# QuanjianSong/UniVST

Hardware: AMD Instinct MI355X
Metric: stylized frames/sec, SD-v1.5 16x512x512 @50 DDIM steps (higher is better)
Workload: dtype f16; 1 GPU; sd15_unet_three_branch_pnp_transfer_16x512x512_50ddim; frames=16, branches=3, schedule_steps=54 (wrapping modulo 50), masks=moving disc, blended on steps 0..45, parallelism=single, weights=random-init SD-v1.5 architecture (859M + 201M temporal params), fp16

## Files before the change

### univst_amd/csrc/attention.hip

```cpp
#include "common.h"

#include "kernels.h"

namespace {

constexpr int KT = 64;
constexpr float DEFER = 8.f;

typedef __fp16 fh2 __attribute__((ext_vector_type(2)));

__device__ __forceinline__ float max3f(float a, float b, float c) {
    float r;
    asm("v_max3_f32 %0, %1, %2, %3" : "=v"(r) : "v"(a), "v"(b), "v"(c));
    return r;
}

__device__ __forceinline__ void attn_merge_coef(float m1, float l1, float m2, float l2, float& w1, float& w2) {
    const bool has1 = l1 > 0.f, has2 = l2 > 0.f;
    const float m = has1 ? (has2 ? fmaxf(m1, m2) : m1) : m2;
    const float a1 = has1 ? l1 * __builtin_amdgcn_exp2f(m1 - m) : 0.f;
    const float a2 = has2 ? __builtin_amdgcn_exp2f(m2 - m) : 0.f;
    const float den = a1 + l2 * a2;
    const float inv = den > 0.f ? 1.f / den : 0.f;
    w1 = a1 * inv;
// ... 721 lines not shown
#define UV_PP_PHASE2()                                                            \
    _Pragma("unroll") for (int i_ = 0; i_ < 12; ++i_) {                           \
        __builtin_amdgcn_sched_group_barrier(0x008, 1, 0);                        \
        if (i_ < 4) __builtin_amdgcn_sched_group_barrier(0x100, 1, 0);            \
        __builtin_amdgcn_sched_group_barrier(0x002, 2, 0);                        \
    }

#define UV_PP_PIN4(a) asm volatile("" : "+v"(a[0]), "+v"(a[1]), "+v"(a[2]), "+v"(a[3]))
#define UV_PP_PIN2(a, i) asm volatile("" : "+v"(a[i]), "+v"(a[(i) + 1]))

    if (STG) {
        dma_tile(0);
        if (T > 1) dma_tile(TILE);
        asm volatile("s_waitcnt vmcnt(0)" ::: "memory");
    } else {
        load_tile();
        store_tile(smem);
        if (T > 1) {
            load_tile();
            store_tile(smem + TILE);
        }
    }
    __syncthreads();

    f4 scA[2][QB], scB[2][QB];
    h8 kf[2][2], vf[DV16], pb[QB];
    float mx[QB];
    int nx_s = 0, nx_t = (ntile > 1) ? 1 : 0;
    if (ntile == 1) nx_s = 1;
    float lw_nxt = (nx_s != 0 && nx_s < nsrc_eff && p.src_logw) ? p.src_logw[bf * p.nsrc + nx_s] : lw_cur;
    int t0_cur = 0, t0_nxt = nx_t * KT;
    half_t* b_cur = smem;
    half_t* b_nxt = smem + TILE;
    half_t* b_ld = smem + 2 * TILE;

    kfrag_read(b_cur, 0, kf);
    qk(kf, scA);
    if (t0_cur + KT > p.Nkv) mask_tail(scA, t0_cur);
    local_max(scA, mx);
    decide(scA, mx, true);
    kfrag_read(b_cur, 1, kf);

    for (int tt = 0; tt < T; ++tt) {
        const bool has_next = tt + 1 < T;
        if (tt + 2 < T) {
            if (STG) dma_tile((int)(b_ld - smem));
            else load_tile();
        }
        vfrag_read(b_cur, 0, vf);
        if (K16) {
            qk_a(kf, scB);
            exp_half(scA, pb, 0);
            UV_PP_PIN2(pb, 0);
            UV_PP_PHASE1H(1);
            qk_fence(scB);
            __builtin_amdgcn_sched_barrier(0);
            qk_b(kf, scB);
            exp_half(scA, pb, 1);
            UV_PP_PIN2(pb, 2);
            UV_PP_PHASE1H(0);
        } else {
            qk(kf, scB);
            exp_part(scA, pb);
            UV_PP_PIN4(pb);
            UV_PP_PHASE1();
        }
        __builtin_amdgcn_sched_barrier(0);
        if (t0_cur + KT > p.Nkv) mask_tail(scB, t0_cur + 32);
        kfrag_read(b_nxt, 0, kf);
        pv(vf, pb);
        local_max(scB, mx);
        UV_PP_PIN4(mx);
        UV_PP_PHASE2();
        __builtin_amdgcn_sched_barrier(0);
        decide(scB, mx, false);
        if (lw_nxt != lw_cur) set_lw(lw_nxt);
        vfrag_read(b_cur, 1, vf);
        if (K16) {
            qk_a(kf, scA);
            exp_half(scB, pb, 0);
            UV_PP_PIN2(pb, 0);
            UV_PP_PHASE1H(1);
            qk_fence(scA);
            __builtin_amdgcn_sched_barrier(0);
            qk_b(kf, scA);
            exp_half(scB, pb, 1);
            UV_PP_PIN2(pb, 2);
            UV_PP_PHASE1H(0);
        } else {
            qk(kf, scA);
            exp_part(scB, pb);
            UV_PP_PIN4(pb);
            UV_PP_PHASE1();
        }
        __builtin_amdgcn_sched_barrier(0);
        if (has_next && t0_nxt + KT > p.Nkv) mask_tail(scA, t0_nxt);
        kfrag_read(b_nxt, 1, kf);
        pv(vf, pb);
        local_max(scA, mx);
        UV_PP_PIN4(mx);
        UV_PP_PHASE2();
        __builtin_amdgcn_sched_barrier(0);
        if (has_next) decide(scA, mx, false);
        if (!STG && tt + 2 < T) store_tile(b_ld);
        if (STG) asm volatile("s_waitcnt vmcnt(0)" ::: "memory");
        __syncthreads();
        half_t* tb = b_cur; b_cur = b_nxt; b_nxt = b_ld; b_ld = tb;
        t0_cur = t0_nxt;
        lw_cur = lw_nxt;
        if (++nx_t == ntile) {
            nx_t = 0;
            if (++nx_s < nsrc_eff && p.src_logw) lw_nxt = p.src_logw[bf * p.nsrc + nx_s];
        }
        t0_nxt = nx_t * KT;
    }
#undef UV_PP_PHASE1
#undef UV_PP_PHASE1H
#undef UV_PP_PIN2
#undef UV_PP_PIN4
#undef UV_PP_PHASE2

#pragma unroll
    for (int qb = 0; qb < QB; ++qb) {
        const float l = __shfl(o[DV16 - 1][qb][0], 32 + l15, 64);
        float inv = 1.f / l, w1 = 0.f;
        const int qrow = qblk * 64 * NW + wave * 16 * QB + qb * 16 + l15;
        if (qrow >= p.Nq) continue;
        half_t* op = p.o + ((long)bf * p.Nq + qrow) * p.ldo + h * D;
        if constexpr (TP != 0) {
            const float m2 = mrun[qb];
            const long srow = (((long)bf * p.heads + h) * p.Nq + qrow) * 2;
            if constexpr (TP == 1) {
                if (g == 0) *reinterpret_cast<float2*>(p.state_out + srow) = make_float2(m2, l);
            } else {
                const float2 st = *reinterpret_cast<const float2*>(p.state_in + srow);
                attn_merge_coef(st.x, st.y, m2, l, w1, inv);
            }
        }
#pragma unroll
        for (int dv = 0; dv < DV16; ++dv) {
            const int dc = dv * 16 + g * 4;
            if (dc < D) {
                h4 ov;
                if constexpr (TP == 2) {
                    const h4 o1 = *reinterpret_cast<const h4*>(op + dc);
#pragma unroll
                    for (int r = 0; r < 4; ++r) ov[r] = (half_t)fmaf((float)o1[r], w1, o[dv][qb][r] * inv);
                } else {
#pragma unroll
                    for (int r = 0; r < 4; ++r) ov[r] = (half_t)(o[dv][qb][r] * inv);
                }
                *reinterpret_cast<h4*>(op + dc) = ov;
            }
        }
    }
}

template <int TAG = 0, int TP = 0>
__global__ __launch_bounds__(256, 2) void attn_pp64_kernel(AttnParams p) {
    constexpr int D = 64, QB = 4;
    constexpr int NW = 4, DV16 = D / 16, NST = 3;
    constexpr int KS = D / 32;
    constexpr int NDK = D / 8, NPV = D / 8;
    constexpr int RB = NW * 16 * QB;
    constexpr int KPL = 512, VPL = 576;
    constexpr int KAREA = NDK * KPL;
    constexpr int TILE = NDK * KPL + NPV * VPL;
    __shared__ __attribute__((aligned(16))) half_t smem[NST * TILE];

    const int tid = threadIdx.x, lane = tid & 63, wave = tid >> 6;
    const int l15 = lane & 15, g = lane >> 4;
    const int nqb = (p.Nq + RB - 1) / RB;
    const int lid = xcd_remap(blockIdx.x, gridDim.x);
    const int qblk = lid % nqb;
    const int h = p.order ? lid / (nqb * p.BF) : (lid / nqb) % p.heads;
    const int bf = p.order ? (lid / nqb) % p.BF : lid / (nqb * p.heads);
    const h8 zero8 = {0, 0, 0, 0, 0, 0, 0, 0};

    const int ntile = (p.Nkv + KT - 1) / KT;
    const int ntile_x = p.kx ? (p.Nkv_x + KT - 1) / KT : 0;
    const int nsrc_eff = p.src_cnt ? p.src_cnt[bf] : p.nsrc;
    const int nseg = nsrc_eff + (p.kx ? 1 : 0);
    const int T = nsrc_eff * ntile + ntile_x;
    if (TP && T == 0) {
        attn_empty_phase<NW * 16 * QB>(p, bf, h, qblk, D);
        return;
    }
    auto seg_lw = [&](int sidx) { return (sidx < nsrc_eff && p.src_logw) ? p.src_logw[bf * p.nsrc + sidx] : 0.f; };
    auto seg_nkv = [&](int sidx) { return sidx < nsrc_eff ? p.Nkv : p.Nkv_x; };
    auto seg_ntile = [&](int sidx) { return sidx < nsrc_eff ? ntile : ntile_x; };

    h8 qf[QB][KS];
#pragma unroll
    for (int qb = 0; qb < QB; ++qb) {
        const int qrow = qblk * RB + wave * 16 * QB + qb * 16 + l15;
#pragma unroll
        for (int ks = 0; ks < KS; ++ks)
            qf[qb][ks] = (qrow < p.Nq && ks * 32 + g * 8 < D) ? *reinterpret_cast<const h8*>(p.q + ((long)bf * p.Nq + qrow) * p.ldq + h * D + ks * 32 + g * 8) : zero8;
    }

    f4 o[DV16][QB], cfold[QB];
    float mrun[QB], lsum[QB];
    float lw_cur = seg_lw(0);
#pragma unroll
    for (int qb = 0; qb < QB; ++qb) {
        mrun[qb] = 0.f;
        lsum[qb] = 0.f;
        cfold[qb] = f4{lw_cur, lw_cur, lw_cur, lw_cur};
#pragma unroll
        for (int dv = 0; dv < DV16; ++dv) o[dv][qb] = f4{0.f, 0.f, 0.f, 0.f};
    }

    const int wave_u = __builtin_amdgcn_readfirstlane(wave);
    const half_t* const zpage = uv_attn_zero_page;
    const unsigned smem_lds = (unsigned)(size_t)((__attribute__((address_space(3))) half_t*)smem);
    auto glds16 = [](const half_t* src, unsigned lds_byte) {
        unsigned keep;
        asm volatile("s_mov_b32 %0, m0\n\ts_mov_b32 m0, %2\n\ts_nop 0\n\tglobal_load_lds_dwordx4 %1, off\n\ts_mov_b32 m0, %0"
                     : "=&s"(keep) : "v"(src), "s"(lds_byte) : "memory");
    };
    const long xk_delta = p.kx ? (long)(p.kx - p.k) : 0, xv_delta = p.kx ? (long)(p.vx - p.v) : 0;
    int ld_s = 0, ld_t = 0;
    long ld_koff, ld_voff, ld_ld;
    int ld_nkv, ld_ntile;
    {
        const long off = (long)__builtin_amdgcn_readfirstlane(p.src_idx[bf * p.nsrc]) * p.Nkv * p.ldkv + h * D;
        ld_koff = off; ld_voff = off; ld_ld = p.ldkv; ld_nkv = p.Nkv; ld_ntile = ntile;
    }
    auto dma_tile = [&](int stage_half) {
        const int t0 = ld_t * KT;
        const bool rok = t0 + lane < ld_nkv;
        const long roff = (long)(t0 + lane) * ld_ld;
        const half_t* const ksrc = p.k + ld_koff + roff;
        const half_t* const vsrc = p.v + ld_voff + roff;
#pragma unroll
        for (int j = 0; j < (NDK + NPV + NW - 1) / NW; ++j) {
            const int pl = wave_u + NW * j;
            if ((j + 1) * NW <= NDK + NPV || pl < NDK + NPV) {
                const bool isv = pl >= NDK;
                const int c = isv ? pl - NDK : pl;
                const half_t* src = rok ? (isv ? vsrc : ksrc) + c * 8 : zpage;
                const int dst = stage_half + (isv ? KAREA + c * VPL : c * KPL);
                glds16(src, __builtin_amdgcn_readfirstlane(smem_lds + 2u * (unsigned)dst));
            }
        }
        if (++ld_t == ld_ntile) {
            ld_t = 0;
            ++ld_s;
            if (ld_s < nsrc_eff) {
                const long off = (long)__builtin_amdgcn_readfirstlane(p.src_idx[bf * p.nsrc + ld_s]) * p.Nkv * p.ldkv + h * D;
                ld_koff = off; ld_voff = off;
            } else if (ld_s < nseg) {
                const long off = (long)__builtin_amdgcn_readfirstlane(p.x_idx[bf]) * p.Nkv_x * p.ldkv_x + h * D;
                ld_koff = off + xk_delta; ld_voff = off + xv_delta; ld_ld = p.ldkv_x; ld_nkv = p.Nkv_x; ld_ntile = ntile_x;
            }
        }
    };

    const int kf_off = g * KPL + l15 * 8;
    const int vf_off = KAREA + ((l15 & 3) >> 1) * VPL + (g * 4 + (l15 >> 2)) * 8 + (l15 & 1) * 4;
    auto kfrag_read = [&](const half_t* st, int hh, h8 (&kf)[2][KS]) {
#pragma unroll
        for (int kb = 0; kb < 2; ++kb)
#pragma unroll
            for (int ks = 0; ks < KS; ++ks) kf[kb][ks] = *reinterpret_cast<const h8*>(&st[kf_off + (hh * 32 + kb * 16) * 8 + ks * 4 * KPL]);
    };
    auto vfrag_read = [&](const half_t* st, int hh, h8 (&vf)[DV16]) {
#pragma unroll
        for (int dv = 0; dv < DV16; ++dv) {
            const half_t* vp = &st[vf_off + hh * 32 * 8 + dv * 2 * VPL];
            fh4 lo = __builtin_amdgcn_ds_read_tr16_b64_v4f16((__attribute__((address_space(3))) fh4*)(vp));
            fh4 hi = __builtin_amdgcn_ds_read_tr16_b64_v4f16((__attribute__((address_space(3))) fh4*)(vp + 16 * 8));
            h8 a;
            a[0] = (half_t)lo[0]; a[1] = (half_t)lo[1]; a[2] = (half_t)lo[2]; a[3] = (half_t)lo[3];
            a[4] = (half_t)hi[0]; a[5] = (half_t)hi[1]; a[6] = (half_t)hi[2]; a[7] = (half_t)hi[3];
            vf[dv] = a;
        }
    };
    auto qk = [&](const h8 (&kf)[2][KS], f4 (&sc)[2][QB]) {
#pragma unroll
        for (int kb = 0; kb < 2; ++kb)
#pragma unroll
            for (int qb = 0; qb < QB; ++qb) sc[kb][qb] = __builtin_amdgcn_mfma_f32_16x16x32_f16(kf[kb][0], qf[qb][0], cfold[qb], 0, 0, 0);
#pragma unroll
        for (int ks = 1; ks < KS; ++ks)
#pragma unroll
            for (int kb = 0; kb < 2; ++kb)
#pragma unroll
                for (int qb = 0; qb < QB; ++qb) sc[kb][qb] = __builtin_amdgcn_mfma_f32_16x16x32_f16(kf[kb][ks], qf[qb][ks], sc[kb][qb], 0, 0, 0);
    };
    auto exp_part = [&](const f4 (&sc)[2][QB], h8 (&pb)[QB]) {
#pragma unroll
        for (int qb = 0; qb < QB; ++qb) {
            union { fh2 h[4]; h8 v; } u;
#pragma unroll
            for (int kb = 0; kb < 2; ++kb) {
                const float e0 = __builtin_amdgcn_exp2f(sc[kb][qb][0]), e1 = __builtin_amdgcn_exp2f(sc[kb][qb][1]);
                const float e2 = __builtin_amdgcn_exp2f(sc[kb][qb][2]), e3 = __builtin_amdgcn_exp2f(sc[kb][qb][3]);
                u.h[kb * 2] = __builtin_amdgcn_cvt_pkrtz(e0, e1);
                u.h[kb * 2 + 1] = __builtin_amdgcn_cvt_pkrtz(e2, e3);
            }
            pb[qb] = u.v;
        }
    };
    auto row_sums = [&](const h8 (&pb)[QB]) {
        const fh2 one2 = {(__fp16)1.f, (__fp16)1.f};
// ... 225 lines not shown
    half_t* const Vs = smem + NKEY * KSTR;

    const int tid = threadIdx.x, lane = tid & 63, wave = tid >> 6;
    const int l15 = lane & 15, g = lane >> 4;
    const int nchunk = (p.Nq + 128 * NIT - 1) / (128 * NIT);
    const int lid = xcd_remap(blockIdx.x, gridDim.x);
    const int chunk = lid % nchunk;
    const int h = (lid / nchunk) % p.heads;
    const int bf = lid / (nchunk * p.heads);
    const float c = p.q_prescaled ? 1.f : p.scale_log2e;
    const h8 zero8 = {0, 0, 0, 0, 0, 0, 0, 0};

    for (int i = tid * 8; i < NKEY * KSTR + NKEY * VSTR; i += 256 * 8) *reinterpret_cast<h8*>(&smem[i]) = zero8;
    __syncthreads();
    {
        const long kvrow0 = (long)p.src_idx[bf * p.nsrc] * p.Nkv;
        for (int idx = tid; idx < p.Nkv * DCH; idx += 256) {
            const int row = idx / DCH, ch = idx - row * DCH;
            const long off = (kvrow0 + row) * p.ldkv + h * D + ch * 8;
            *reinterpret_cast<h8*>(&Ks[row * KSTR + ch * 8]) = *reinterpret_cast<const h8*>(p.k + off);
            *reinterpret_cast<h8*>(&Vs[row * VSTR + ch * 8]) = *reinterpret_cast<const h8*>(p.v + off);
        }
    }
    __syncthreads();
    h8 kf[NKF][KS];
#pragma unroll
    for (int kfi = 0; kfi < NKF; ++kfi)
#pragma unroll
        for (int ks = 0; ks < KS; ++ks) kf[kfi][ks] = *reinterpret_cast<const h8*>(&Ks[(kfi * 16 + l15) * KSTR + ks * 32 + g * 8]);
    h8 vf[DV16][2];
    h8 vf4[DV16];
    const int vf_off = (g * 4 + (l15 >> 2)) * VSTR + (l15 & 3) * 4;
#pragma unroll
    for (int dv = 0; dv < DV16; ++dv) {
#pragma unroll
        for (int t = 0; t < 2; ++t) {
            const half_t* vp = &Vs[vf_off + t * 32 * VSTR + dv * 16];
            fh4 lo = __builtin_amdgcn_ds_read_tr16_b64_v4f16((__attribute__((address_space(3))) fh4*)(vp));
            fh4 hi = __builtin_amdgcn_ds_read_tr16_b64_v4f16((__attribute__((address_space(3))) fh4*)(vp + 16 * VSTR));
            h8 a;
            a[0] = (half_t)lo[0]; a[1] = (half_t)lo[1]; a[2] = (half_t)lo[2]; a[3] = (half_t)lo[3];
            a[4] = (half_t)hi[0]; a[5] = (half_t)hi[1]; a[6] = (half_t)hi[2]; a[7] = (half_t)hi[3];
            vf[dv][t] = a;
        }
        fh4 lo = __builtin_amdgcn_ds_read_tr16_b64_v4f16((__attribute__((address_space(3))) fh4*)(&Vs[vf_off + 64 * VSTR + dv * 16]));
        h8 b = zero8;
        b[0] = (half_t)lo[0]; b[1] = (half_t)lo[1]; b[2] = (half_t)lo[2]; b[3] = (half_t)lo[3];
        vf4[dv] = b;
    }

    const f4 z = {0.f, 0.f, 0.f, 0.f};
    auto load_q = [&](int q0, h8 (&qf)[2][KS]) {
#pragma unroll
        for (int qb = 0; qb < 2; ++qb) {
            const int qrow = q0 + qb * 16 + l15;
#pragma unroll
            for (int ks = 0; ks < KS; ++ks) {
                const int dc = ks * 32 + g * 8;
                qf[qb][ks] = (qrow < p.Nq && dc < D) ? *reinterpret_cast<const h8*>(p.q + ((long)bf * p.Nq + qrow) * p.ldq + h * D + dc) : zero8;
            }
        }
    };
    h8 qf[2][KS], qn[2][KS];
    load_q(chunk * NIT * 128 + wave * 32, qf);
    for (int it = 0; it < NIT; ++it) {
        const int q0 = (chunk * NIT + it) * 128 + wave * 32;
        if (q0 >= p.Nq) break;
        if (it + 1 < NIT) load_q(q0 + 128, qn);
        f4 sc[NKF][2];
#pragma unroll
        for (int kfi = 0; kfi < NKF; ++kfi)
#pragma unroll
            for (int qb = 0; qb < 2; ++qb) {
                f4 a = __builtin_amdgcn_mfma_f32_16x16x32_f16(kf[kfi][0], qf[qb][0], z, 0, 0, 0);
#pragma unroll
                for (int ks = 1; ks < KS; ++ks) a = __builtin_amdgcn_mfma_f32_16x16x32_f16(kf[kfi][ks], qf[qb][ks], a, 0, 0, 0);
                sc[kfi][qb] = a;
            }
#pragma unroll
        for (int kfi = 0; kfi < NKF; ++kfi)
            if (kfi * 16 + 16 > p.Nkv) {
#pragma unroll
                for (int qb = 0; qb < 2; ++qb)
#pragma unroll
                    for (int r = 0; r < 4; ++r)
                        if (kfi * 16 + g * 4 + r >= p.Nkv) sc[kfi][qb][r] = -INFINITY;
            }
#pragma unroll
        for (int qb = 0; qb < 2; ++qb) {
            float m = max3f(sc[0][qb][0], sc[0][qb][1], sc[0][qb][2]);
            m = max3f(m, sc[0][qb][3], sc[1][qb][0]);
#pragma unroll
            for (int kfi = 1; kfi < NKF; ++kfi) {
                m = max3f(m, sc[kfi][qb][1], sc[kfi][qb][2]);
                m = max3f(m, sc[kfi][qb][3], kfi + 1 < NKF ? sc[kfi + 1][qb][0] : sc[kfi][qb][3]);
            }
            const float o16 = __shfl_xor(m, 16, 64);
            m = max3f(m, o16, o16);
            const float o32 = __shfl_xor(m, 32, 64);
            m = max3f(m, o32, o32);
            const float mc = -m * c;
            float l = 0.f;
            union { fh2 h2v[4]; h8 v; } u0, u1;
            union { fh2 h2v[4]; h8 v; } u2;
            u2.v = zero8;
#pragma unroll
            for (int kfi = 0; kfi < NKF; ++kfi) {
                const float e0 = __builtin_amdgcn_exp2f(fmaf(sc[kfi][qb][0], c, mc)), e1 = __builtin_amdgcn_exp2f(fmaf(sc[kfi][qb][1], c, mc));
                const float e2 = __builtin_amdgcn_exp2f(fmaf(sc[kfi][qb][2], c, mc)), e3 = __builtin_amdgcn_exp2f(fmaf(sc[kfi][qb][3], c, mc));
                const fh2 p01 = __builtin_amdgcn_cvt_pkrtz(e0, e1), p23 = __builtin_amdgcn_cvt_pkrtz(e2, e3);
                l += ((float)p01[0] + (float)p01[1]) + ((float)p23[0] + (float)p23[1]);
                if (kfi == 0) { u0.h2v[0] = p01; u0.h2v[1] = p23; }
                else if (kfi == 1) { u0.h2v[2] = p01; u0.h2v[3] = p23; }
                else if (kfi == 2) { u1.h2v[0] = p01; u1.h2v[1] = p23; }
                else if (kfi == 3) { u1.h2v[2] = p01; u1.h2v[3] = p23; }
                else { u2.h2v[0] = p01; u2.h2v[1] = p23; }
            }
            l += __shfl_xor(l, 16, 64);
            l += __shfl_xor(l, 32, 64);
            const float inv = 1.f / l;
            const int qrow = q0 + qb * 16 + l15;
            half_t* op = p.o + ((long)bf * p.Nq + qrow) * p.ldo + h * D;
#pragma unroll
            for (int dv = 0; dv < DV16; ++dv) {
                f4 o = __builtin_amdgcn_mfma_f32_16x16x32_f16(vf[dv][0], u0.v, z, 0, 0, 0);
                o = __builtin_amdgcn_mfma_f32_16x16x32_f16(vf[dv][1], u1.v, o, 0, 0, 0);
                o = __builtin_amdgcn_mfma_f32_16x16x32_f16(vf4[dv], u2.v, o, 0, 0, 0);
                const int dc = dv * 16 + g * 4;
                if (qrow < p.Nq && dc < D) {
                    h4 ov;
#pragma unroll
                    for (int r = 0; r < 4; ++r) ov[r] = (half_t)(o[r] * inv);
                    *reinterpret_cast<h4*>(op + dc) = ov;
                }
            }
        }
#pragma unroll
        for (int qb = 0; qb < 2; ++qb)
#pragma unroll
            for (int ks = 0; ks < KS; ++ks) qf[qb][ks] = qn[qb][ks];
    }
}

template <int DPAD, int DV16, int QB>
__global__ __launch_bounds__(256, 2) void attn_kernel_occ2(AttnParams p) {
    attn_body<DPAD, DV16, QB>(p);
}

template <int DPAD, int DV16, int TP>
int launch_attn_tp(const AttnParams& p, hipStream_t stream) {
    if constexpr (DPAD == 64 && DV16 == 3) {
        if (p.q_prescaled && p.Nq >= 2048) {
            const int nqb4 = (p.Nq + 255) / 256;
            hipLaunchKernelGGL((attn_pp40_kernel<0, 1, true, TP>), dim3(nqb4 * p.heads * p.BF), dim3(256), 0, stream, p);
            UV_LAUNCH_CHECK();
            return UV_OK;
        }
    }
    if constexpr (DPAD == 64 && DV16 == 4) {
        if (p.q_prescaled && (p.Nq >= 1024 || ((p.kx || TP == 2) && p.Nq >= 192))) {
            const int nqb4 = (p.Nq + 255) / 256;
            hipLaunchKernelGGL((attn_pp64_kernel<0, TP>), dim3(nqb4 * p.heads * p.BF), dim3(256), 0, stream, p);
            UV_LAUNCH_CHECK();
            return UV_OK;
        }
    }
    const int QB = p.Nq >= 512 ? 2 : 1;
    const int nqb = (p.Nq + 64 * QB - 1) / (64 * QB);
    dim3 grid(nqb * p.heads * p.BF), block(256);
    if constexpr (DPAD >= 96) {
        if (p.q_prescaled) {
            if (QB == 2) {
                if constexpr (DPAD == 96) hipLaunchKernelGGL((attn_kernel_occ3<DPAD, DV16, 2, true, TP>), grid, block, 0, stream, p);
                else hipLaunchKernelGGL((attn_kernel<DPAD, DV16, 2, true, TP>), grid, block, 0, stream, p);
            } else {
                hipLaunchKernelGGL((attn_kernel<DPAD, DV16, 1, true, TP>), grid, block, 0, stream, p);
            }
            UV_LAUNCH_CHECK();
            return UV_OK;
        }
    }
    if (QB == 2) {
        if constexpr (DPAD <= 96) hipLaunchKernelGGL((attn_kernel_occ3<DPAD, DV16, 2, false, TP>), grid, block, 0, stream, p);
        else hipLaunchKernelGGL((attn_kernel<DPAD, DV16, 2, false, TP>), grid, block, 0, stream, p);
    } else {
        hipLaunchKernelGGL((attn_kernel<DPAD, DV16, 1, false, TP>), grid, block, 0, stream, p);
    }
    UV_LAUNCH_CHECK();
    return UV_OK;
}

template <int DPAD, int DV16>
int launch_attn(const AttnParams& p, hipStream_t stream) {
    if (p.state_out) return launch_attn_tp<DPAD, DV16, 1>(p, stream);
    if (p.state_in) return launch_attn_tp<DPAD, DV16, 2>(p, stream);
    if constexpr (DPAD == 64 && DV16 == 3) {
        if (!p.kx && p.Nq >= 2048 && p.q_prescaled) {
            const int nqb4 = (p.Nq + 255) / 256;
            if (p.nsrc == 1 && p.Nkv <= 128) hipLaunchKernelGGL((attn_pp40_kernel<1>), dim3(nqb4 * p.heads * p.BF), dim3(256), 0, stream, p);
            else hipLaunchKernelGGL((attn_pp40_kernel<0, 1, true>), dim3(nqb4 * p.heads * p.BF), dim3(256), 0, stream, p);
            UV_LAUNCH_CHECK();
            return UV_OK;
        }
    }
    if constexpr (DPAD == 64 && DV16 == 4) {
        if (p.q_prescaled && (p.Nq >= 1024 || (p.kx && p.Nq >= 192))) {
            const int nqb4 = (p.Nq + 255) / 256;
            hipLaunchKernelGGL((attn_pp64_kernel<0>), dim3(nqb4 * p.heads * p.BF), dim3(256), 0, stream, p);
            UV_LAUNCH_CHECK();
            return UV_OK;
        }
    }
    if constexpr (DPAD <= 64) {
        if (p.Nq >= 2048) {
            const int nqb4 = (p.Nq + 255) / 256;
            hipLaunchKernelGGL((attn_kernel_occ2<DPAD, DV16, 4>), dim3(nqb4 * p.heads * p.BF), dim3(256), 0, stream, p);
            UV_LAUNCH_CHECK();
            return UV_OK;
        }
    }
    const int QB = p.Nq >= 512 ? 2 : 1;
    const int nqb = (p.Nq + 64 * QB - 1) / (64 * QB);
    dim3 grid(nqb * p.heads * p.BF), block(256);
    if constexpr (DPAD >= 96) {
        if (p.q_prescaled) {
            if constexpr (DPAD == 96) {
                if (QB == 2) hipLaunchKernelGGL((attn_kernel_occ3<DPAD, DV16, 2, true>), grid, block, 0, stream, p);
                else hipLaunchKernelGGL((attn_kernel<DPAD, DV16, 1, true>), grid, block, 0, stream, p);
            } else {
                if (QB == 2) hipLaunchKernelGGL((attn_kernel<DPAD, DV16, 2, true>), grid, block, 0, stream, p);
                else hipLaunchKernelGGL((attn_kernel<DPAD, DV16, 1, true>), grid, block, 0, stream, p);
            }
            UV_LAUNCH_CHECK();
            return UV_OK;
        }
    }
    if constexpr (DPAD <= 96) {
        if (QB == 2) {
            hipLaunchKernelGGL((attn_kernel_occ3<DPAD, DV16, 2>), grid, block, 0, stream, p);
            UV_LAUNCH_CHECK();
            return UV_OK;
        }
    }
    if (QB == 2) hipLaunchKernelGGL((attn_kernel<DPAD, DV16, 2>), grid, block, 0, stream, p);
    else hipLaunchKernelGGL((attn_kernel<DPAD, DV16, 1>), grid, block, 0, stream, p);
    UV_LAUNCH_CHECK();
    return UV_OK;
}

}

static int attn_dispatch(const AttnParams& p, hipStream_t stream);

int uv_launch_attention(const AttnParams& p0, hipStream_t stream) {
    AttnParams p = p0;
    p.order = 1;
    UV_REQUIRE(p.d % 8 == 0, "attention: head_dim=%d must be a multiple of 8", p.d);
    UV_REQUIRE(p.nsrc >= 1 && p.Nkv >= 1 && p.Nq >= 1, "attention: empty problem");
    UV_REQUIRE(p.ldq % 8 == 0 && p.ldkv % 8 == 0 && p.ldo % 4 == 0, "attention: row strides must be multiples of 8");
    UV_REQUIRE(!p.kx || (p.vx && p.x_idx && p.Nkv_x >= 1 && p.ldkv_x % 8 == 0), "attention: extra key segment needs vx, x_idx, Nkv_x >= 1 and a row stride that is a multiple of 8");
    UV_REQUIRE(!(p.state_out && p.state_in), "attention: a launch is the first phase (state_out) or the merge phase (state_in) of a two-phase attention, not both");
    const double nkv = (double)p.nsrc * p.Nkv;
    const int cls = (p.nsrc == 1 && p.Nkv <= 128) ? UV_CLS_ATTN_TEXT
                    : (p.d == 40 && p.Nq >= 2048) ? UV_CLS_ATTN_D40 : (p.d == 80 ? UV_CLS_ATTN_D80 : UV_CLS_ATTN_OTHER);
    uv_prof_begin(cls, p.state_in ? 0.0 : 4.0 * p.BF * p.heads * (double)p.Nq * nkv * p.d,
                  2.0 * p.BF * p.heads * p.d * (2.0 * p.Nq + (p.state_in ? 0.0 : 2.0 * nkv)), stream);
    int rc = attn_dispatch(p, stream);
    uv_prof_end(stream);
    return rc;
}

static int attn_dispatch(const AttnParams& p, hipStream_t stream) {
    if (!p.kx && !p.state_out && !p.state_in && p.nsrc == 1 && p.Nkv <= 80 && !p.src_logw && (p.d == 40 || p.d == 80) && p.Nq >= 256) {
        const int nchunk = (p.Nq + 1023) / 1024;
        const dim3 grid((unsigned)(nchunk * p.heads * p.BF));
        if (p.d == 40) hipLaunchKernelGGL((attn_text_kernel<40>), grid, dim3(256), 0, stream, p);
        else hipLaunchKernelGGL((attn_text_kernel<80>), grid, dim3(256), 0, stream, p);
        UV_LAUNCH_CHECK();
        return UV_OK;
    }
    switch (p.d) {

        case 16: return launch_attn<32, 1>(p, stream);
        case 32: return launch_attn<32, 2>(p, stream);
        case 40: return launch_attn<64, 3>(p, stream);
        case 64: return launch_attn<64, 4>(p, stream);
        case 80: return launch_attn<96, 5>(p, stream);
        case 160: return launch_attn<160, 10>(p, stream);
        default:
            uv_set_error("attention: head_dim=%d not instantiated (16,32,40,64,80,160)", p.d);
            return UV_ERR_UNSUPPORTED;
    }
}

int uv_launch_tr16_probe(float* out, hipStream_t stream) {
    hipLaunchKernelGGL(tr16_probe_kernel, dim3(1), dim3(64), 0, stream, out);
    UV_LAUNCH_CHECK();
    return UV_OK;
}
```

Baseline: 6.040 frames/s.

## Add 32x32x16 MFMA head-dim-40 flash attention kernel with software-pipelined QK/PV

Adds a new attention kernel for head dimension 40 that uses 32x32x16 MFMA tiles and folds the running-max shift and log-weight bias into extra Q/K columns. It keeps a three-stage LDS ring fed by direct global-to-LDS loads, and interleaves QK, exp and PV of alternating half-tiles under explicit scheduling barriers. Softmax rescaling is deferred until the max grows past a threshold. The new kernel replaces the previous head-dim-40 path for large query counts and for stateful (split) attention. It adds register pressure and the deferral adds numeric risk, with the old kernel kept only for very short KV sequences.

```diff
diff --git a/univst_amd/csrc/attention.hip b/univst_amd/csrc/attention.hip
--- a/univst_amd/csrc/attention.hip
+++ b/univst_amd/csrc/attention.hip
@@ -897,6 +897,337 @@
                 }
                 *reinterpret_cast<h4*>(op + dc) = ov;
             }
+        }
+    }
+}
+
+typedef float f16x __attribute__((ext_vector_type(16)));
+
+template <int TP = 0>
+__global__ __launch_bounds__(256, 2) void attn_pp40w_kernel(AttnParams p) {
+    constexpr int NW = 4, D = 40, DCH = D / 8, QB = 2, NST = 3;
+    constexpr int KPL = 512, VPL = 544;
+    constexpr int KAREA = 6 * KPL;
+    constexpr int TILE = KAREA + 8 * VPL;
+    __shared__ __attribute__((aligned(16))) half_t smem[NST * TILE];
+
+    const int tid = threadIdx.x, lane = tid & 63, wave = tid >> 6;
+    const int l31 = lane & 31, hf = lane >> 5, l15 = lane & 15;
+    const int nqb = (p.Nq + 64 * NW - 1) / (64 * NW);
+    const int lid = xcd_remap(blockIdx.x, gridDim.x);
+    const int qblk = lid % nqb;
+    const int h = p.order ? lid / (nqb * p.BF) : (lid / nqb) % p.heads;
+    const int bf = p.order ? (lid / nqb) % p.BF : lid / (nqb * p.heads);
+    const h8 zero8 = {0, 0, 0, 0, 0, 0, 0, 0};
+
+    const int ntile = (p.Nkv + KT - 1) / KT;
+    const int nsrc_eff = p.src_cnt ? p.src_cnt[bf] : p.nsrc;
+    const int T = nsrc_eff * ntile;
+    if (TP && T == 0) {
+        attn_empty_phase<64 * NW>(p, bf, h, qblk, D);
+        return;
+    }
+    float lw_cur = p.src_logw ? p.src_logw[bf * p.nsrc] : 0.f;
+
+    h8 qf[QB][3];
+#pragma unroll
+    for (int qb = 0; qb < QB; ++qb) {
+        const int qrow = qblk * 64 * NW + wave * 64 + qb * 32 + l31;
+#pragma unroll
+        for (int ks = 0; ks < 3; ++ks) {
+            const int dc = ks * 16 + hf * 8;
+            qf[qb][ks] = (qrow < p.Nq && dc < D) ? *reinterpret_cast<const h8*>(p.q + ((long)bf * p.Nq + qrow) * p.ldq + h * D + dc) : zero8;
+        }
+        if (hf == 1) qf[qb][2][2] = (half_t)lw_cur;
+    }
+    auto set_shift = [&](int qb, float M) -> float {
+        const float hi = floorf(M * 0.125f) * 8.f, lo = M - hi;
+        const half_t hh = (half_t)(-hi), lh = (half_t)(-lo);
+        if (hf == 1) {
+            qf[qb][2][0] = hh;
+            qf[qb][2][1] = lh;
+        }
+        return -((float)hh + (float)lh);
+    };
+
+    f16x o[2][QB];
+    float mrun[QB];
+#pragma unroll
+    for (int qb = 0; qb < QB; ++qb) {
+        mrun[qb] = 0.f;
+#pragma unroll
+        for (int dt = 0; dt < 2; ++dt)
+#pragma unroll
+            for (int r = 0; r < 16; ++r) o[dt][qb][r] = 0.f;
+    }
+
+    const int wave_u = __builtin_amdgcn_readfirstlane(wave);
+    int ld_s = 0, ld_t = 0;
+    long ld_off = (long)__builtin_amdgcn_readfirstlane(p.src_idx[bf * p.nsrc]) * p.Nkv * p.ldkv;
+    auto advance_ld = [&]() {
+        if (++ld_t == ntile) {
+            ld_t = 0;
+            if (++ld_s < nsrc_eff) ld_off = (long)__builtin_amdgcn_readfirstlane(p.src_idx[bf * p.nsrc + ld_s]) * p.Nkv * p.ldkv;
+        }
+    };
+    const half_t* const zpage = uv_attn_zero_page;
+    const unsigned smem_lds = (unsigned)(size_t)((__attribute__((address_space(3))) half_t*)smem);
+    auto glds16 = [](const half_t* src, unsigned lds_byte) {
+        unsigned keep;
+        asm volatile("s_mov_b32 %0, m0\n\ts_mov_b32 m0, %2\n\ts_nop 0\n\tglobal_load_lds_dwordx4 %1, off\n\ts_mov_b32 m0, %0"
+                     : "=&s"(keep) : "v"(src), "s"(lds_byte) : "memory");
+    };
+    constexpr int NDJ = (2 * DCH + NW - 1) / NW;
+    const half_t* dma_src[NDJ];
+    unsigned dma_dst[NDJ];
+#pragma unroll
+    for (int j = 0; j < NDJ; ++j) {
+        const int pl = wave_u + NW * j;
+        const bool isv = pl >= DCH;
+        const int c = isv ? pl - DCH : pl;
+        dma_src[j] = (isv ? p.v : p.k) + h * D + c * 8 + (long)lane * p.ldkv;
+        dma_dst[j] = smem_lds + 2u * (unsigned)(isv ? KAREA + c * VPL : c * KPL);
+    }
+    auto dma_tile = [&](int stage_half) {
+        const int t0 = ld_t * KT;
+        const bool rok = t0 + lane < p.Nkv;
+        const long roff = ld_off + (long)t0 * p.ldkv;
+#pragma unroll
+        for (int j = 0; j < NDJ; ++j) {
+            if ((j + 1) * NW <= 2 * DCH || wave_u + NW * j < 2 * DCH)
+                glds16(rok ? dma_src[j] + roff : zpage, __builtin_amdgcn_readfirstlane(dma_dst[j] + 2u * (unsigned)stage_half));
+        }
+        advance_ld();
+    };
+    {
+        for (int i = tid * 8; i < NST * TILE; i += NW * 64 * 8) *reinterpret_cast<h8*>(&smem[i]) = zero8;
+        __syncthreads();
+        if (tid < KT) {
+#pragma unroll
+            for (int st = 0; st < NST; ++st) {
+                smem[st * TILE + KAREA + 5 * VPL + tid * 8] = (half_t)1.f;
+                smem[st * TILE + 5 * KPL + tid * 8] = (half_t)1.f;
+                smem[st * TILE + 5 * KPL + tid * 8 + 1] = (half_t)1.f;
+                smem[st * TILE + 5 * KPL + tid * 8 + 2] = (half_t)1.f;
+            }
+        }
+        __syncthreads();
+    }
+
+    const int kf_off = hf * KPL + l31 * 8;
+    const int vf_off = KAREA + (((lane >> 4) & 1) * 2 + ((l15 & 3) >> 1)) * VPL + (hf * 4 + (l15 >> 2)) * 8 + (l15 & 1) * 4;
+    auto kfrag_read = [&](const half_t* st, int hh, h8 (&kf)[3]) {
+#pragma unroll
+        for (int ks = 0; ks < 3; ++ks) kf[ks] = *reinterpret_cast<const h8*>(&st[kf_off + hh * 32 * 8 + ks * 2 * KPL]);
+    };
+    auto vfrag_read = [&](const half_t* st, int hh, h8 (&vf)[2][2]) {
+#pragma unroll
+        for (int dt = 0; dt < 2; ++dt)
+#pragma unroll
+            for (int kk = 0; kk < 2; ++kk) {
+                const half_t* vp = &st[vf_off + dt * 4 * VPL + (hh * 32 + kk * 16) * 8];
+                fh4 lo = __builtin_amdgcn_ds_read_tr16_b64_v4f16((__attribute__((address_space(3))) fh4*)(vp));
+                fh4 hi = __builtin_amdgcn_ds_read_tr16_b64_v4f16((__attribute__((address_space(3))) fh4*)(vp + 8 * 8));
+                h8 a;
+                a[0] = (half_t)lo[0]; a[1] = (half_t)lo[1]; a[2] = (half_t)lo[2]; a[3] = (half_t)lo[3];
+                a[4] = (half_t)hi[0]; a[5] = (half_t)hi[1]; a[6] = (half_t)hi[2]; a[7] = (half_t)hi[3];
+                vf[dt][kk] = a;
+            }
+    };
+    auto qk = [&](const h8 (&kf)[3], f16x (&sc)[QB]) {
+        f16x z;
+#pragma unroll
+        for (int r = 0; r < 16; ++r) z[r] = 0.f;
+#pragma unroll
+        for (int ks = 0; ks < 3; ++ks)
+#pragma unroll
+            for (int qb = 0; qb < QB; ++qb) sc[qb] = __builtin_amdgcn_mfma_f32_32x32x16_f16(kf[ks], qf[qb][ks], ks ? sc[qb] : z, 0, 0, 0);
+    };
+    auto exp_part = [&](const f16x (&sc)[QB], h8 (&pb)[QB][2]) {
+#pragma unroll
+        for (int kk = 0; kk < 2; ++kk)
+#pragma unroll
+            for (int qb = 0; qb < QB; ++qb) {
+                union { fh2 h[4]; h8 v; } u;
+#pragma unroll
+                for (int i = 0; i < 4; ++i)
+                    u.h[i] = __builtin_amdgcn_cvt_pkrtz(__builtin_amdgcn_exp2f(sc[qb][kk * 8 + 2 * i]), __builtin_amdgcn_exp2f(sc[qb][kk * 8 + 2 * i + 1]));
+                pb[qb][kk] = u.v;
+            }
+    };
+    auto pv = [&](const h8 (&vf)[2][2], const h8 (&pb)[QB][2]) {
+#pragma unroll
+        for (int kk = 0; kk < 2; ++kk)
+#pragma unroll
+            for (int dt = 0; dt < 2; ++dt)
+#pragma unroll
+                for (int qb = 0; qb < QB; ++qb) o[dt][qb] = __builtin_amdgcn_mfma_f32_32x32x16_f16(vf[dt][kk], pb[qb][kk], o[dt][qb], 0, 0, 0);
+    };
+    auto local_max = [&](const f16x (&sc)[QB], float (&mx)[QB]) {
+#pragma unroll
+        for (int qb = 0; qb < QB; ++qb) {
+            float m = max3f(sc[qb][0], sc[qb][1], sc[qb][2]);
+#pragma unroll
+            for (int r = 3; r < 15; r += 2) m = max3f(m, sc[qb][r], sc[qb][r + 1]);
+            mx[qb] = max3f(m, sc[qb][15], sc[qb][15]);
+        }
+    };
+    auto mask_tail = [&](f16x (&sc)[QB], int key0) {
+#pragma unroll
+        for (int qb = 0; qb < QB; ++qb)
+#pragma unroll
+            for (int r = 0; r < 16; ++r)
+                if (key0 + (r >> 2) * 8 + hf * 4 + (r & 3) >= p.Nkv) sc[qb][r] = -INFINITY;
+    };
+    auto decide = [&](f16x (&sc)[QB], const float (&mx)[QB], bool first) {
+        if (!first) {
+            if (__builtin_amdgcn_ballot_w64(fmaxf(mx[0], mx[1]) > DEFER) == 0) return;
+        }
+#pragma unroll
+        for (int qb = 0; qb < QB; ++qb) {
+            if (__builtin_amdgcn_ballot_w64(first || mx[qb] > DEFER) != 0) {
+                float m = mx[qb];
+                const float o32 = __shfl_xor(m, 32, 64);
+                m = max3f(m, o32, o32);
+                float delta = floorf(m * 64.f + 0.5f) * (1.f / 64.f);
+                if (!first) delta = fmaxf(delta, 0.f);
+                const float mnew = set_shift(qb, mrun[qb] + delta);
+                delta = mnew - mrun[qb];
+                mrun[qb] = mnew;
+                const float alpha = first ? 1.f : __builtin_amdgcn_exp2f(-delta);
+#pragma unroll
+                for (int r = 0; r < 16; ++r) sc[qb][r] -= delta;
+#pragma unroll
+                for (int r = 0; r < 16; ++r) o[0][qb][r] *= alpha;
+#pragma unroll
+                for (int r = 0; r < 5; ++r) o[1][qb][r] *= alpha;
+            }
+        }
+    };
+    auto set_lw = [&](float lw) {
+        if (hf == 1) {
+#pragma unroll
+            for (int qb = 0; qb < QB; ++qb) qf[qb][2][2] = (half_t)lw;
+        }
+    };
+#define UV_PW_PHASE1()                                                            \
+    _Pragma("unroll") for (int i_ = 0; i_ < 6; ++i_) {                            \
+        __builtin_amdgcn_sched_group_barrier(0x008, 1, 0);                        \
+        if (i_ < 4) __builtin_amdgcn_sched_group_barrier(0x100, 2, 0);            \
+        _Pragma("unroll") for (int j_ = 0; j_ < 3; ++j_) {                        \
+            __builtin_amdgcn_sched_group_barrier(0x400, 2, 0);                    \
+            __builtin_amdgcn_sched_group_barrier(0x002, 1, 0);                    \
+        }                                                                         \
+    }
+#define UV_PW_PHASE2()                                                            \
+    _Pragma("unroll") for (int i_ = 0; i_ < 8; ++i_) {                            \
+        __builtin_amdgcn_sched_group_barrier(0x008, 1, 0);                        \
+        if (i_ < 3) __builtin_amdgcn_sched_group_barrier(0x100, 1, 0);            \
+        __builtin_amdgcn_sched_group_barrier(0x002, 2, 0);                        \
+    }
+#define UV_PW_PINP(a) asm volatile("" : "+v"(a[0][0]), "+v"(a[0][1]), "+v"(a[1][0]), "+v"(a[1][1]))
+#define UV_PW_PINM(a) asm volatile("" : "+v"(a[0]), "+v"(a[1]))
+
+    dma_tile(0);
+    if (T > 1) dma_tile(TILE);
+    asm volatile("s_waitcnt vmcnt(0)" ::: "memory");
+    __syncthreads();
+
+    f16x scA[QB], scB[QB];
+    h8 kf[3], vf[2][2], pb[QB][2];
+    float mx[QB];
+    int nx_s = 0, nx_t = (ntile > 1) ? 1 : 0;
+    if (ntile == 1) nx_s = 1;
+    float lw_nxt = (nx_s != 0 && nx_s < nsrc_eff && p.src_logw) ? p.src_logw[bf * p.nsrc + nx_s] : lw_cur;
+    int t0_cur = 0, t0_nxt = nx_t * KT;
+    half_t* b_cur = smem;
+    half_t* b_nxt = smem + TILE;
+    half_t* b_ld = smem + 2 * TILE;
+
+    kfrag_read(b_cur, 0, kf);
+    qk(kf, scA);
+    if (t0_cur + KT > p.Nkv) mask_tail(scA, t0_cur);
+    local_max(scA, mx);
+    decide(scA, mx, true);
+    kfrag_read(b_cur, 1, kf);
+
+    for (int tt = 0; tt < T; ++tt) {
+        const bool has_next = tt + 1 < T;
+        if (tt + 2 < T) dma_tile((int)(b_ld - smem));
+        vfrag_read(b_cur, 0, vf);
+        qk(kf, scB);
+        exp_part(scA, pb);
+        UV_PW_PINP(pb);
+        UV_PW_PHASE1();
+        __builtin_amdgcn_sched_barrier(0);
+        if (t0_cur + KT > p.Nkv) mask_tail(scB, t0_cur + 32);
+        kfrag_read(b_nxt, 0, kf);
+        pv(vf, pb);
+        local_max(scB, mx);
+        UV_PW_PINM(mx);
+        UV_PW_PHASE2();
+        __builtin_amdgcn_sched_barrier(0);
+        decide(scB, mx, false);
+        if (lw_nxt != lw_cur) set_lw(lw_nxt);
+        vfrag_read(b_cur, 1, vf);
+        qk(kf, scA);
+        exp_part(scB, pb);
+        UV_PW_PINP(pb);
+        UV_PW_PHASE1();
+        __builtin_amdgcn_sched_barrier(0);
+        if (has_next && t0_nxt + KT > p.Nkv) mask_tail(scA, t0_nxt);
+        kfrag_read(b_nxt, 1, kf);
+        pv(vf, pb);
+        local_max(scA, mx);
+        UV_PW_PINM(mx);
+        UV_PW_PHASE2();
+        __builtin_amdgcn_sched_barrier(0);
+        if (has_next) decide(scA, mx, false);
+        asm volatile("s_waitcnt vmcnt(0)" ::: "memory");
+        __syncthreads();
+        half_t* tb = b_cur; b_cur = b_nxt; b_nxt = b_ld; b_ld = tb;
+        t0_cur = t0_nxt;
+        lw_cur = lw_nxt;
+        if (++nx_t == ntile) {
+            nx_t = 0;
+            if (++nx_s < nsrc_eff && p.src_logw) lw_nxt = p.src_logw[bf * p.nsrc + nx_s];
+        }
+        t0_nxt = nx_t * KT;
+    }
+#undef UV_PW_PHASE1
+#undef UV_PW_PHASE2
+#undef UV_PW_PINP
+#undef UV_PW_PINM
+
+#pragma unroll
+    for (int qb = 0; qb < QB; ++qb) {
+        const float l = __shfl(o[1][qb][4], l31, 64);
+        float inv = 1.f / l, w1 = 0.f;
+        const int qrow = qblk * 64 * NW + wave * 64 + qb * 32 + l31;
+        if (qrow >= p.Nq) continue;
+        half_t* op = p.o + ((long)bf * p.Nq + qrow) * p.ldo + h * D;
+        if constexpr (TP != 0) {
+            const float m2 = mrun[qb];
+            const long srow = (((long)bf * p.heads + h) * p.Nq + qrow) * 2;
+            if constexpr (TP == 1) {
+                if (hf == 0) *reinterpret_cast<float2*>(p.state_out + srow) = make_float2(m2, l);
+            } else {
+                const float2 st = *reinterpret_cast<const float2*>(p.state_in + srow);
+                attn_merge_coef(st.x, st.y, m2, l, w1, inv);
+            }
+        }
+#pragma unroll
+        for (int b = 0; b < 5; ++b) {
+            const int dc = b * 8 + hf * 4;
+            h4 ov, o1 = {0, 0, 0, 0};
+            if constexpr (TP == 2) o1 = *reinterpret_cast<const h4*>(op + dc);
+#pragma unroll
+            for (int r = 0; r < 4; ++r) {
+                const float acc = b < 4 ? o[0][qb][b * 4 + r] : o[1][qb][r];
+                if constexpr (TP == 2) ov[r] = (half_t)fmaf((float)o1[r], w1, acc * inv);
+                else ov[r] = (half_t)(acc * inv);
+            }
+            *reinterpret_cast<h4*>(op + dc) = ov;
         }
     }
 }
@@ -1428,7 +1759,7 @@
     if constexpr (DPAD == 64 && DV16 == 3) {
         if (p.q_prescaled && p.Nq >= 2048) {
             const int nqb4 = (p.Nq + 255) / 256;
-            hipLaunchKernelGGL((attn_pp40_kernel<0, 1, true, TP>), dim3(nqb4 * p.heads * p.BF), dim3(256), 0, stream, p);
+            hipLaunchKernelGGL((attn_pp40w_kernel<TP>), dim3(nqb4 * p.heads * p.BF), dim3(256), 0, stream, p);
             UV_LAUNCH_CHECK();
             return UV_OK;
         }
@@ -1474,7 +1805,8 @@
         if (!p.kx && p.Nq >= 2048 && p.q_prescaled) {
             const int nqb4 = (p.Nq + 255) / 256;
             if (p.nsrc == 1 && p.Nkv <= 128) hipLaunchKernelGGL((attn_pp40_kernel<1>), dim3(nqb4 * p.heads * p.BF), dim3(256), 0, stream, p);
-            else hipLaunchKernelGGL((attn_pp40_kernel<0, 1, true>), dim3(nqb4 * p.heads * p.BF), dim3(256), 0, stream, p);
+            else if (p.nsrc * ((p.Nkv + KT - 1) / KT) < 4) hipLaunchKernelGGL((attn_pp40_kernel<0, 1, true>), dim3(nqb4 * p.heads * p.BF), dim3(256), 0, stream, p);
+            else hipLaunchKernelGGL((attn_pp40w_kernel<0>), dim3(nqb4 * p.heads * p.BF), dim3(256), 0, stream, p);
             UV_LAUNCH_CHECK();
             return UV_OK;
         }
```

New measurement: 5.917 frames/s, median of 2. 0.98x the previous value.
